# imazen/codec-eval

Hardware: AMD Instinct MI355X
Metric: metric MP/s (SSIMULACRA2+DSSIM+Butteraugli) at 1/2/4/8 GPU; HBM-roofline % (higher is better)
Workload: dtype f32

## Files before the change

### codec-eval_amd/csrc/ce_api.cpp

```cpp
#include <algorithm>
#include <atomic>
#include <condition_variable>
#include <functional>
#include <mutex>
#include <thread>
#include <cmath>
#include <cstdlib>
#include <cstring>
#include <new>

#include "ce_internal.h"

namespace {

thread_local std::string g_err_noctx;

int fail(ce_ctx *ctx, int code, const std::string &msg)
{
    if (ctx) ctx->err = msg; else g_err_noctx = msg;
    return code;
}

int bad_length(ce_ctx *ctx, size_t want, size_t got)
{
// ... 475 lines not shown
        if (b->h_stage[k]) hipHostFree(b->h_stage[k]);
        if (b->ev_stage[k]) hipEventDestroy(b->ev_stage[k]);
    }
    for (int l = 0; l < 3; l++) {
        if (b->metric_stream[l]) hipStreamSynchronize(b->metric_stream[l]);
        if (b->ev_join[l]) hipEventDestroy(b->ev_join[l]);
    }
    ce_ssim2_free(b);
    ce_dssim_free(b);
    ce_butteraugli_free(b);
    delete b;
}

static void invalidate_reference_state(ce_batch *b)
{
    b->ssim2_ref_src = nullptr;
    b->ds_ref_src = nullptr;
    b->ba_ref_src = nullptr;
    b->refs_rt_valid = false;
}

static bool is_pinned_host(const void *p)
{
    hipPointerAttribute_t a{};
    if (hipPointerGetAttributes(&a, p) != hipSuccess) {
        (void)hipGetLastError();
        return false;
    }
    return a.type == hipMemoryTypeHost;
}

// ... 530 lines not shown

int ce_batch_run(ce_batch *b, uint32_t n_pairs, uint32_t metric_mask, uint32_t flags, float intensity_target,
                 ce_scores *out)
{
    if (int rc = ce_batch_launch(b, n_pairs, metric_mask, flags, intensity_target)) return rc;
    return ce_batch_collect(b, n_pairs, out);
}


size_t ce_estimate_batch_bytes(uint32_t w, uint32_t h, uint32_t n_refs, uint32_t n_pairs, uint32_t metric_mask)
{
    const double px = (double)w * h, slots = (double)n_refs + n_pairs, pairs = n_pairs;
    double bytes = 3.0 * px * slots + 64.0 * pairs;
    double allocations = 8;
    if (metric_mask & CE_METRIC_SSIMULACRA2) {
        bytes += px * (20.0 * slots + 80.0 * pairs);
        allocations += 24;
    }
    if (metric_mask & CE_METRIC_DSSIM) {
        bytes += px * (6.0 * slots + 48.0 * n_refs + 17.4 * pairs);
        allocations += 24;
    }
    if (metric_mask & CE_METRIC_BUTTERAUGLI) {
        bytes += px * (91.0 * slots + 10.0 * n_refs + 1.0 * pairs);
        allocations += 20;
    }
    if (metric_mask & CE_METRIC_PSNR) bytes += 8.0 * pairs;
    return (size_t)(bytes * 1.2) + (size_t)(allocations * (256u << 10)) + (8u << 20);
}

size_t ce_estimate_batch_bytes_deep(uint32_t w, uint32_t h, uint32_t n_refs, uint32_t n_pairs, uint32_t metric_mask, uint32_t ref_depth,
                                    uint32_t test_depth)
// ... 770 lines not shown
```

### codec-eval_amd/csrc/ce_internal.h

```cpp
#pragma once

#include <hip/hip_runtime.h>

#include <cstdint>
#include <cstdio>
#include <map>
#include <string>
#include <tuple>
#include <utility>
#include <vector>

#include "ce_metrics.h"
#include "ce_metrics_debug.h"
#include "ce_plan.h"

#define CE_MAX_SCALES 6
#define CE_SSIM2_STREAMS 5
#define CE_DSSIM_SCALES 5
enum { CE_SRC_F32 = 0, CE_SRC_U8 = 1, CE_SRC_U16 = 2 };
static_assert(CE_MAX_SCALES == CE_SSIM2_MAX_SCALES, "the ABI's scale count is the pyramid's");

struct ce_scale_dims {
    uint32_t w, h, pitch;
    size_t plane;
// ... 90 lines not shown
    hipStream_t up_stream = nullptr;
    hipEvent_t ev_up = nullptr, ev_run = nullptr;
    bool uploads_pending = false, run_pending = false;
    bool inline_pending = false;
    bool counted_in_flight = false;
    uint8_t *h_wide[2] = {}, *d_wide[2] = {};
    hipEvent_t ev_wide[2] = {};
    bool wide_busy[2] = {};
    int next_wide = 0;

    int n_scales = 0;
    ce_scale_dims sd[CE_MAX_SCALES];
    float *d_lin[CE_MAX_SCALES] = {};
    float *d_xyb[CE_MAX_SCALES] = {};
    float *d_hbuf[CE_MAX_SCALES] = {};
    hipStream_t lvl_stream[CE_MAX_SCALES] = {};
    hipStream_t metric_stream[3] = {};
    hipEvent_t ev_fork = nullptr, ev_join[3] = {};
    hipEvent_t ev_prep[CE_MAX_SCALES] = {}, ev_done[CE_MAX_SCALES] = {};
    double *d_partials = nullptr;
    uint32_t max_vblocks = 0;
    double *d_avg = nullptr;
    float *s2_map = nullptr;
    float *s2_map_lvl[CE_MAX_SCALES] = {};
    uint32_t s2_map_pairs = 0, s2_norm_pairs = 0, s2_scales_run = 0;
    float *s2_cells = nullptr;
    size_t s2_cells_cap = 0;
    ce_dev_scores *d_scores = nullptr;
    ce_dev_scores *h_scores = nullptr;
    bool ssim2_ready = false;
    ce_xcd_list work_h, work_v;
    ce_xcd_list work_ht, work_vt;
    bool keep_ref_pyramid = false;
    const uint8_t *ssim2_ref_src = nullptr;
    uint32_t ssim2_ref_count = 0;
    int ssim2_ref_levels = 0;
    bool refs_rt_valid = false;
    int debug_max_scales = CE_MAX_SCALES;
    uint32_t ref_builds[3] = {0, 0, 0};

    struct dssim_level { uint32_t w, h, pitch; size_t plane; };
    int ds_levels = 0;
    dssim_level ds[CE_DSSIM_SCALES];
    float *ds_lin[2] = {};
    float *ds_img = nullptr;
    float *ds_rimg[CE_DSSIM_SCALES] = {}, *ds_rmu[CE_DSSIM_SCALES] = {}, *ds_rsq[CE_DSSIM_SCALES] = {};
    const uint8_t *ds_ref_src = nullptr;
    uint32_t ds_ref_count = 0;
    float *ds_map = nullptr;
    double *ds_part = nullptr;
    double *ds_level_scores = nullptr;
// ... 122 lines not shown
```

### codec-eval_amd/csrc/ce_plan.h

```cpp
#pragma once

#include <algorithm>
#include <cstdint>
#include <map>
#include <vector>

inline constexpr uint32_t ce_plan_ring_slots = 3;
inline constexpr size_t ce_plan_none = ~(size_t)0;

struct ce_plan_inputs {
    size_t budget;
    size_t per_pair;
    uint32_t pooled_pairs;
    size_t forced_chunks;
    size_t ramp;
};

struct ce_plan_chunk {
    uint32_t slot;
    uint32_t max_pairs;
    size_t collect_first;
    std::vector<std::vector<size_t>> refs;
};

// ... 27 lines not shown
        for (size_t p = bucket_begin; p < plan.size(); p++)
            if (plan[p].slot == c.slot) c.collect_first = p;
        plan.push_back(std::move(c));
    }
}

struct ce_plan_entry {
    uint32_t tile, pair;
};

struct ce_xcd_keys {
    uint32_t channels;
    uint32_t keys_per_channel;
    uint32_t tiles_per_key;
    uint32_t round_to = 1;
};

inline bool operator==(const ce_xcd_keys &a, const ce_xcd_keys &b)
{
    return a.channels == b.channels && a.keys_per_channel == b.keys_per_channel && a.tiles_per_key == b.tiles_per_key &&
           a.round_to == b.round_to;
}

inline std::vector<ce_plan_entry> ce_plan_xcd_list(const uint32_t *pair_ref, uint32_t n_pairs, uint32_t n_refs, const ce_xcd_keys &k)
{
    std::vector<std::vector<uint32_t>> pairs_of(n_refs);
    for (uint32_t p = 0; p < n_pairs; p++) pairs_of[pair_ref[p]].push_back(p);
    std::vector<ce_plan_entry> cls[8];
    uint32_t key = 0;
    for (const auto &pairs : pairs_of) {
        if (pairs.empty()) continue;
        for (uint32_t c = 0; c < k.channels; c++)
            for (uint32_t j = 0; j < k.keys_per_channel; j++, key++)
                for (uint32_t sub = 0; sub < k.tiles_per_key; sub++)
                    for (uint32_t p : pairs) cls[key & 7].push_back({(j * k.tiles_per_key + sub) | c << 16, p});
    }
    size_t len = 0;
    for (const auto &v : cls) len = std::max(len, v.size());
    len = (len + k.round_to - 1) / k.round_to * k.round_to;
    std::vector<ce_plan_entry> list(len * 8, ce_plan_entry{~0u, 0u});
    for (uint32_t x = 0; x < 8; x++)
        for (size_t i = 0; i < cls[x].size(); i++) list[i * 8 + x] = cls[x][i];
    return list;
}

inline uint32_t ce_plan_dssim_levels(uint32_t w, uint32_t h, uint32_t max_levels, uint32_t *level_w, uint32_t *level_h)
{
    if (w == 0 || h == 0) return 0;
    uint32_t n = 0;
    while (n < max_levels) {
// ... 26 lines not shown
```

### codec-eval_amd/csrc/ssim2.hip

```cpp
#include <algorithm>
#include <cstdlib>

#include "ce_internal.h"

namespace {

struct rg_consts {
    float mul_in[3];
    float mul_prev[3];
};

constexpr int kColsPerBlock = 64;

constexpr int kTailLevels = CE_MAX_SCALES - 1;
struct lvl_table {
    uint32_t n, first_level;
    uint32_t blk_end[kTailLevels];
    uint32_t w[kTailLevels], h[kTailLevels], pitch[kTailLevels];
    size_t plane[kTailLevels];
    const float *xyb[kTailLevels];
    float *hbuf[kTailLevels];
};

__device__ __forceinline__ uint32_t slot_of(uint32_t z, uint32_t n_refs_used, uint32_t max_refs)
{
    return z < n_refs_used ? z : max_refs + (z - n_refs_used);
}

__device__ __noinline__ float cbrt_f32_exact(float x)
{
    uint32_t hx = __float_as_uint(x) & 0x7fffffffu;
    if (hx == 0) return x;
    float t;
    if (hx < 0x00800000u) {
        t = __uint_as_float(0x4b800000u) * x;
        t = __uint_as_float((__float_as_uint(t) & 0x7fffffffu) / 3 + 642849266u);
// ... 283 lines not shown
                float *dst = base + l_dst[m];
                const bool rv = l_row[m] < h && col >= 0;
                dst[0] = (rv && col < (int)w) ? pf[m].x : 0.0f;
                dst[HB_LD] = (rv && col + 1 < (int)w) ? pf[m].y : 0.0f;
                dst[2 * HB_LD] = (rv && col + 2 < (int)w) ? pf[m].z : 0.0f;
                dst[3 * HB_LD] = (rv && col + 3 < (int)w) ? pf[m].w : 0.0f;
            }
        }
    };

    load_chunk(0);
    stash_chunk(0);
    if (n_chunks > 1) load_chunk(1);
    __syncthreads();

    const bool full = pair_first[p] == p;
    const uint32_t n_jobs = full ? CE_SSIM2_STREAMS : 3;
    const bool worker = tid < n_jobs * HB_ROWS;
    const uint32_t tj = worker ? tid / HB_ROWS : 0, tr = worker ? tid % HB_ROWS : 0;
    const uint32_t ts = full ? tj : (tj == 0 ? 1u : tj + 2u);
    const bool plain = ts < 2;
    const float *sp = &s_in[(ts == 1 || ts == 3) ? 1 : 0][tr];
    const float *sq = &s_in[(ts == 2) ? 0 : 1][tr];
    float *so = &s_out[ts * HB_HALF + tr];
    hblur_state st;
    st.p01 = st.q01 = hb_f2{0.0f, 0.0f};
    st.p2 = st.q2 = 0.0f;
#pragma unroll
    for (int j = 0; j < 10; j++) st.d[j] = 0.0f;
    float *obase = hbuf + ((size_t)p * 3 + c) * CE_SSIM2_STREAMS * plane;

// ... 16 lines not shown
                    *reinterpret_cast<float4 *>(obase + (size_t)os * plane + (size_t)(y0 + orow) * pitch + HB_CW * (k - 1) + 4 * oq) = v;
            }
        }
        lds_barrier();
    }
}

__device__ __forceinline__ double wave_sum(double v)
{
#pragma unroll
    for (int off = 32; off > 0; off >>= 1) v += __shfl_down(v, off, 64);
    return v;
}

constexpr int VB_G = 4;
constexpr int VB_PLANES = 7;
constexpr int VB_SLOT = VB_G * 64;
constexpr int VB_GROUP = VB_PLANES * VB_SLOT;

struct vblur_state {
    float prev[CE_SSIM2_STREAMS][3], prev2[CE_SSIM2_STREAMS][3];
    float rr[16][CE_SSIM2_STREAMS];
    double acc[6];
};

template <int GG, bool CHECKED, bool STORE>
__device__ __forceinline__ void vblur_group(vblur_state &st, const float *__restrict__ slot, int g, uint32_t h,
                                            const rg_consts &rg, float *__restrict__ map, uint32_t pitch, size_t plane,
                                            uint32_t lane, bool active)
{
    const float C2 = 0.0009f;
    float gacc[6] = {0.f, 0.f, 0.f, 0.f, 0.f, 0.f};
#pragma unroll
    for (int e = 0; e < VB_G; e++) {
        const uint32_t i = (uint32_t)(4 * g + e);
        constexpr int base = 4 * GG;
        const int re = base + e;
        float v[CE_SSIM2_STREAMS];
#pragma unroll
        for (int s = 0; s < CE_SSIM2_STREAMS; s++) {
            const float ld = slot[s * VB_SLOT + e * 64];
            const float right = (!CHECKED || i < h) ? ld : 0.0f;
            const float left = st.rr[(re + 6) & 15][s];
            st.rr[re][s] = right;
            v[s] = rg_step(left + right, st.prev[s], st.prev2[s], rg);
        }
        if (!CHECKED || (i >= 4 && i < h + 4)) {
            const float img1 = slot[5 * VB_SLOT + e * 64], img2 = slot[6 * VB_SLOT + e * 64];
            const float mu1 = v[0], mu2 = v[1], s11 = v[2], s22 = v[3], s12 = v[4];
            const float mu11 = mu1 * mu1, mu22 = mu2 * mu2, mu12 = mu1 * mu2;
            const float mu_diff = mu1 - mu2;
            const float num_m = __builtin_fmaf(mu_diff, -mu_diff, 1.0f);
            const float num_s = __builtin_fmaf(2.0f, s12 - mu12, C2);
            const float denom_s = (s11 - mu11) + (s22 - mu22) + C2;
            float d = 1.0f - (num_m * num_s) / denom_s;
            d = d > 0.0f ? d : 0.0f;
            const float dd = d * d;
            const float e1 = fabsf(img1 - mu1), e2 = fabsf(img2 - mu2);
            const float d1 = (e2 - e1) * __builtin_amdgcn_rcpf(1.0f + e1);
            const float artifact = d1 > 0.0f ? d1 : 0.0f;
            const float detail = d1 < 0.0f ? -d1 : 0.0f;
            const float aa = artifact * artifact, ll = detail * detail;
            if (STORE && active) {
                float *row = map + (size_t)(i - 4) * pitch;
// ... 1 lines not shown
                (row + plane)[lane] = artifact;
                (row + 2 * plane)[lane] = detail;
            }
            gacc[0] += d;
            gacc[1] += dd * dd;
            gacc[2] += artifact;
            gacc[3] += aa * aa;
            gacc[4] += detail;
            gacc[5] += ll * ll;
        }
    }
#pragma unroll
    for (int q = 0; q < 6; q++) st.acc[q] += (double)gacc[q];
}

struct ssim2_map_table {
    float *lvl[CE_MAX_SCALES];
};

template <int LEVEL, bool STORE>
__global__ __launch_bounds__(64) void k_ssim2_vblur_dma(const float *__restrict__ hbuf, const float *__restrict__ xyb,
                                                        const uint32_t *__restrict__ pair_ref,
                                                        double *__restrict__ partials, uint32_t w, uint32_t h,
                                                        uint32_t pitch, size_t plane, uint32_t max_refs, uint32_t scale,
                                                        uint32_t max_vblocks, rg_consts rg, lvl_table tab,
                                                        const uint2 *__restrict__ work, const uint32_t *__restrict__ pair_first,
                                                        ssim2_map_table maps)
{
    __shared__ __attribute__((aligned(16))) float ring[2 * VB_GROUP];
    uint32_t bx = blockIdx.x, c = blockIdx.y, p = blockIdx.z;
    if (work) {
        const uint2 wi = work[blockIdx.x];
        if (wi.x == ~0u) return;
        bx = wi.x & 0xffffu, c = wi.x >> 16, p = wi.y;
    }
    if (LEVEL < 0) {
        uint32_t l = 0;
        while (l + 1 < tab.n && bx >= tab.blk_end[l]) l++;
        bx -= l ? tab.blk_end[l - 1] : 0;
        xyb = tab.xyb[l], hbuf = tab.hbuf[l];
        w = tab.w[l], h = tab.h[l], pitch = tab.pitch[l], plane = tab.plane[l];
        scale = tab.first_level + l;
    }
    const uint32_t lane = threadIdx.x, x0 = bx * 64;
    const bool active = x0 + lane < w;
    const float *hb = hbuf + ((size_t)p * 3 + c) * CE_SSIM2_STREAMS * plane + x0;
    const float *hb_ref = hbuf + ((size_t)pair_first[p] * 3 + c) * CE_SSIM2_STREAMS * plane + x0;
    const float *xa = xyb + ((size_t)pair_ref[p] * 3 + c) * plane + x0;
    const float *xb = xyb + ((size_t)(max_refs + p) * 3 + c) * plane + x0;
    const uint32_t dr = lane >> 4, dc = (lane & 15) * 4;
    float *map = STORE ? maps.lvl[scale] + ((size_t)p * 9 + (size_t)c * 3) * plane + x0 : nullptr;

    using gptr = const __attribute__((address_space(1))) void *;
    using lptr = __attribute__((address_space(3))) void *;
    auto issue_group = [&](int g) {
        float *dst = ring + (g & 1) * VB_GROUP;
        const uint32_t row = min((uint32_t)(4 * g) + dr, h - 1);
        const size_t off = (size_t)row * pitch + dc;
#pragma unroll
        for (int s = 0; s < CE_SSIM2_STREAMS; s++)
            __builtin_amdgcn_global_load_lds((gptr)(((s == 0 || s == 2) ? hb_ref : hb) + (size_t)s * plane + off), (lptr)(dst + s * VB_SLOT), 16, 0, 0);
        const int rx = 4 * g - 4 + (int)dr;
        const size_t offx = (size_t)min((uint32_t)max(rx, 0), h - 1) * pitch + dc;
        __builtin_amdgcn_global_load_lds((gptr)(xa + offx), (lptr)(dst + 5 * VB_SLOT), 16, 0, 0);
        __builtin_amdgcn_global_load_lds((gptr)(xb + offx), (lptr)(dst + 6 * VB_SLOT), 16, 0, 0);
    };

    vblur_state st;
#pragma unroll
    for (int s = 0; s < CE_SSIM2_STREAMS; s++) {
#pragma unroll
        for (int k = 0; k < 3; k++) st.prev[s][k] = st.prev2[s][k] = 0.0f;
#pragma unroll
        for (int e = 0; e < 16; e++) st.rr[e][s] = 0.0f;
    }
#pragma unroll
    for (int q = 0; q < 6; q++) st.acc[q] = 0.0;
    const int n_groups = (int)((h + 4 + VB_G - 1) / VB_G);
    const int full_groups = (int)(h / VB_G);

    issue_group(0);
    issue_group(1);
#define CE_VGROUP(GG, CHECKED)                                                                         \
    do {                                                                                               \
                    \
        asm volatile("s_waitcnt vmcnt(7)" ::: "memory");                                               \
        vblur_group<GG, CHECKED, STORE>(st, ring + ((GG) & 1) * VB_GROUP + lane, g0 + (GG), h, rg, map, \
                                        pitch, plane, lane, active);                                   \
                      \
        asm volatile("s_waitcnt lgkmcnt(0)" ::: "memory");                                             \
        issue_group(g0 + (GG) + 2);                                                                    \
    } while (0)
    int g0 = 0;
    {
        CE_VGROUP(0, true);
        CE_VGROUP(1, true);
        if (2 < n_groups) CE_VGROUP(2, true);
        if (3 < n_groups) CE_VGROUP(3, true);
        g0 = 4;
    }
    for (; g0 + 3 < full_groups; g0 += 4) {
        CE_VGROUP(0, false);
        CE_VGROUP(1, false);
        CE_VGROUP(2, false);
        CE_VGROUP(3, false);
    }
    for (; g0 < n_groups; g0 += 4) {
        CE_VGROUP(0, true);
        if (g0 + 1 < n_groups) CE_VGROUP(1, true);
        if (g0 + 2 < n_groups) CE_VGROUP(2, true);
        if (g0 + 3 < n_groups) CE_VGROUP(3, true);
    }
#undef CE_VGROUP
    asm volatile("s_waitcnt vmcnt(0)" ::: "memory");
    double *dst = partials + ((((size_t)p * CE_MAX_SCALES + scale) * 3 + c) * max_vblocks + bx) * 6;
#pragma unroll
    for (int q = 0; q < 6; q++) {
        const double sum = wave_sum(active ? st.acc[q] : 0.0);
        if (lane == 0) dst[q] = sum;
    }
}

__global__ __launch_bounds__(256) void k_cbrt_sweep(uint32_t first, uint64_t count, unsigned long long *out)
{
    uint64_t mism = 0, slow = 0;
    for (uint64_t i = (uint64_t)blockIdx.x * blockDim.x + threadIdx.x; i < count; i += (uint64_t)gridDim.x * blockDim.x) {
        const float x = __uint_as_float(first + (uint32_t)i);
// ... 61 lines not shown
        else
            ssim = 100.0;
        scores[p].ssimulacra2 = ssim;
    }
}

}


void ce_ssim2_free(ce_batch *b)
{
    for (int s = 0; s < CE_MAX_SCALES; s++) {
        hipFree(b->d_lin[s]);
        hipFree(b->d_xyb[s]);
        hipFree(b->d_hbuf[s]);
        b->d_lin[s] = b->d_xyb[s] = b->d_hbuf[s] = nullptr;
        if (b->lvl_stream[s]) hipStreamSynchronize(b->lvl_stream[s]);
        if (b->ev_prep[s]) hipEventDestroy(b->ev_prep[s]);
        if (b->ev_done[s]) hipEventDestroy(b->ev_done[s]);
        b->lvl_stream[s] = nullptr;
        b->ev_prep[s] = b->ev_done[s] = nullptr;
    }
    hipFree(b->d_partials);
    hipFree(b->d_avg);
    hipFree(b->s2_map);
    hipFree(b->s2_cells);
    b->d_partials = nullptr;
    b->d_avg = nullptr;
    b->s2_map = b->s2_cells = nullptr;
    for (int s = 0; s < CE_MAX_SCALES; s++) b->s2_map_lvl[s] = nullptr;
    b->s2_cells_cap = 0;
    b->s2_map_pairs = b->s2_norm_pairs = 0;
    for (ce_xcd_list *L : {&b->work_h, &b->work_v, &b->work_ht, &b->work_vt}) ce_free_xcd_list(L);
    b->ssim2_ready = false;
}

static int ssim2_allocate(ce_batch *b)
{
    ce_ctx *ctx = b->ctx;
    const int ns = b->n_scales;
    const size_t slots = (size_t)b->max_refs + b->max_pairs;
    for (int s = 1; s < ns; s++)
        CE_HIP(ctx, hipMalloc(&b->d_lin[s], slots * 3 * b->sd[s].plane * sizeof(float)));
    for (int s = 0; s < ns; s++) {
        CE_HIP(ctx, hipMalloc(&b->d_xyb[s], slots * 3 * b->sd[s].plane * sizeof(float)));
        CE_HIP(ctx, hipMalloc(&b->d_hbuf[s], (size_t)b->max_pairs * 3 * CE_SSIM2_STREAMS * b->sd[s].plane * sizeof(float)));
        if (s == 0 && !(b->lvl_stream[0] = ce_ctx_aux_stream(ctx, ce_ctx::AUX_SSIM2_L0))) return CE_ERR_BACKEND;
        CE_HIP(ctx, hipEventCreateWithFlags(&b->ev_prep[s], hipEventDisableTiming));
        CE_HIP(ctx, hipEventCreateWithFlags(&b->ev_done[s], hipEventDisableTiming));
    }
    b->max_vblocks = (b->sd[0].w + kColsPerBlock - 1) / kColsPerBlock;
    CE_HIP(ctx, hipMalloc(&b->d_partials, (size_t)b->max_pairs * CE_MAX_SCALES * 3 * b->max_vblocks * 6 * sizeof(double)));
    CE_HIP(ctx, hipMalloc(&b->d_avg, (size_t)b->max_pairs * CE_MAX_SCALES * 18 * sizeof(double)));
    return CE_OK;
}

int ce_ssim2_prepare(ce_batch *b)
{
    if (b->ssim2_ready) return CE_OK;
    uint32_t sw[CE_MAX_SCALES], sh[CE_MAX_SCALES];
    const int ns = (int)ce_plan_ssim2_scales(b->w, b->h, CE_MAX_SCALES, sw, sh);
// ... 9 lines not shown
    }
    b->n_scales = ns;
    if (ns == 0) return CE_OK;
    const int rc = ssim2_allocate(b);
    if (rc != CE_OK) {
        const std::string why = b->ctx->err;
        ce_ssim2_free(b);
        (void)hipGetLastError();
        b->ctx->err = why;
        return rc;
    }
    b->ssim2_ready = true;
    return CE_OK;
}

static int build_pass_list(ce_batch *b, uint32_t n_pairs, uint32_t n_blocks, ce_xcd_list *L)
{
    if (n_blocks > 0xffffu) {
        b->ctx->err = "SSIMULACRA2: image too large for the block index of the work list";
        return CE_ERR_INVALID_ARG;
    }
    return ce_build_xcd_list(b, n_pairs, ce_xcd_keys{3, n_blocks, 1}, L);
}

int ce_launch_ssim2(ce_batch *b, const uint8_t *d_refs, uint32_t n_refs_used, uint32_t n_pairs, bool store_maps)
{
    ce_ctx *ctx = b->ctx;
    int rc = ce_ssim2_prepare(b);
    if (rc != CE_OK) return rc;
    ssim2_map_table maps{};
    if (store_maps) {
        if (!b->s2_map) {
            size_t total = 0;
            for (int s = 0; s < b->n_scales; s++) total += (size_t)b->max_pairs * 9 * b->sd[s].plane;
            if (hipMalloc(&b->s2_map, total * sizeof(float)) != hipSuccess) {
                b->s2_map = nullptr;
                (void)hipGetLastError();
// ... 3 lines not shown
            size_t off = 0;
            for (int s = 0; s < b->n_scales; s++) {
                b->s2_map_lvl[s] = b->s2_map + off;
                off += (size_t)b->max_pairs * 9 * b->sd[s].plane;
            }
        }
        for (int s = 0; s < b->n_scales; s++) maps.lvl[s] = b->s2_map_lvl[s];
    }
    rg_consts rg;
    ce_ssim2_recursive_gaussian(rg.mul_in, rg.mul_prev);
    const uint32_t n_slots = n_refs_used + n_pairs;
    const bool cached = b->keep_ref_pyramid && b->ssim2_ref_src == d_refs && b->ssim2_ref_count >= n_refs_used &&
                        b->ssim2_ref_levels == std::min(b->n_scales, b->debug_max_scales);
    const uint32_t z0 = cached ? n_refs_used : 0;
    if (!cached) b->ref_builds[0]++;
    using hblur_fn = void (*)(const float *, const uint32_t *, float *, uint32_t, uint32_t, uint32_t, size_t, uint32_t,
                              rg_consts, lvl_table, const uint2 *, const uint32_t *);
    using vblur_fn = void (*)(const float *, const float *, const uint32_t *, double *, uint32_t, uint32_t, uint32_t,
                              size_t, uint32_t, uint32_t, uint32_t, rg_consts, lvl_table, const uint2 *, const uint32_t *,
                              ssim2_map_table);
    const hblur_fn h_l0 = k_ssim2_hblur_lds<0>, h_tail = k_ssim2_hblur_lds<-1>;
    const vblur_fn v_l0 = k_ssim2_vblur_dma<0, false>, v_tail = k_ssim2_vblur_dma<-1, false>;
    const vblur_fn v_l0_map = k_ssim2_vblur_dma<0, true>, v_tail_map = k_ssim2_vblur_dma<-1, true>;
    scale_geom g{};
    const int levels = std::min(b->n_scales, b->debug_max_scales);
    hipStream_t s0 = ctx->prof_serial ? CE_STREAM(ctx) : b->lvl_stream[0];
    hipStream_t s1 = CE_STREAM(ctx);
    lvl_table tab{};
    lvl_table tab_v{};
    for (int s = 0; s < levels; s++) {
        const ce_scale_dims &d = b->sd[s];
        const bool has_next = s + 1 < levels;
        const ce_scale_dims &nd = b->sd[has_next ? s + 1 : s];
        const dim3 quad_grid(((d.w + 1) / 2 + 63) / 64, ((d.h + 1) / 2 + 3) / 4, n_slots - z0);
// ... 8 lines not shown
        else
            CE_LAUNCH(ctx, "ssim2_prep", k_ssim2_prep<CE_SRC_F32>, quad_grid, dim3(256), 0, d_refs, b->d_tests, ctx->d_lut_ssim2, ctx->d_lut_ssim2,
                      (const float *)b->d_lin[s], b->d_xyb[s], b->d_lin[has_next ? s + 1 : s], d.w, d.h, d.pitch, d.plane,
                      nd.pitch, nd.plane, has_next ? 1 : 0, b->img_bytes, n_refs_used, b->max_refs, z0);
        const uint32_t hblk = (d.h + HB_ROWS - 1) / HB_ROWS, vblk = (d.w + kColsPerBlock - 1) / kColsPerBlock;
        g.npix[s] = d.w * d.h;
        g.nblk[s] = vblk;
        if (s == 0) {
            if (s0 != CE_STREAM(ctx)) {
                CE_HIP(ctx, hipEventRecord(b->ev_prep[0], CE_STREAM(ctx)));
                CE_HIP(ctx, hipStreamWaitEvent(s0, b->ev_prep[0], 0));
            }
            if ((rc = build_pass_list(b, n_pairs, hblk, &b->work_h)) != CE_OK) return rc;
            if ((rc = build_pass_list(b, n_pairs, vblk, &b->work_v)) != CE_OK) return rc;
            CE_LAUNCH_ON(ctx, s0, "ssim2_hblur_L0", h_l0, dim3(b->work_h.len), dim3(HB_THREADS), 0, b->d_xyb[0], b->d_pair_ref,
                         b->d_hbuf[0], d.w, d.h, d.pitch, d.plane, b->max_refs, rg, tab, (const uint2 *)b->work_h.d,
                         (const uint32_t *)b->d_pair_first);
#define CE_VBLUR_L0_ARGS                                                                                                   \
    b->d_hbuf[0], b->d_xyb[0], b->d_pair_ref, b->d_partials, d.w, d.h, d.pitch, d.plane, b->max_refs, 0u, b->max_vblocks, rg, tab, \
        (const uint2 *)b->work_v.d, (const uint32_t *)b->d_pair_first, maps
            if (store_maps)
                CE_LAUNCH_ON(ctx, s0, "ssim2_vblur_ssim_map_L0", v_l0_map, dim3(b->work_v.len), dim3(64), 0, CE_VBLUR_L0_ARGS);
            else
                CE_LAUNCH_ON(ctx, s0, "ssim2_vblur_ssim_L0", v_l0, dim3(b->work_v.len), dim3(64), 0, CE_VBLUR_L0_ARGS);
#undef CE_VBLUR_L0_ARGS
            if (s0 != CE_STREAM(ctx)) CE_HIP(ctx, hipEventRecord(b->ev_done[0], s0));
        } else {
            const uint32_t l = tab.n++;
            tab_v.n = tab.n;
            tab.first_level = tab_v.first_level = 1;
            tab.blk_end[l] = (l ? tab.blk_end[l - 1] : 0) + hblk;
            tab_v.blk_end[l] = (l ? tab_v.blk_end[l - 1] : 0) + vblk;
            tab.w[l] = tab_v.w[l] = d.w;
            tab.h[l] = tab_v.h[l] = d.h;
            tab.pitch[l] = tab_v.pitch[l] = d.pitch;
            tab.plane[l] = tab_v.plane[l] = d.plane;
            tab.xyb[l] = tab_v.xyb[l] = b->d_xyb[s];
            tab.hbuf[l] = tab_v.hbuf[l] = b->d_hbuf[s];
        }
    }
    if (tab.n) {
        if (s1 != CE_STREAM(ctx)) {
            CE_HIP(ctx, hipEventRecord(b->ev_prep[1], CE_STREAM(ctx)));
            CE_HIP(ctx, hipStreamWaitEvent(s1, b->ev_prep[1], 0));
        }
        if ((rc = build_pass_list(b, n_pairs, tab.blk_end[tab.n - 1], &b->work_ht)) != CE_OK) return rc;
        if ((rc = build_pass_list(b, n_pairs, tab_v.blk_end[tab_v.n - 1], &b->work_vt)) != CE_OK) return rc;
        CE_LAUNCH_ON(ctx, s1, "ssim2_hblur_L1-5", h_tail, dim3(b->work_ht.len), dim3(HB_THREADS), 0,
                     (const float *)nullptr, b->d_pair_ref, (float *)nullptr, 0u, 0u, 0u, (size_t)0, b->max_refs, rg, tab,
                     (const uint2 *)b->work_ht.d, (const uint32_t *)b->d_pair_first);
#define CE_VBLUR_TAIL_ARGS                                                                                                  \
    (const float *)nullptr, (const float *)nullptr, b->d_pair_ref, b->d_partials, 0u, 0u, 0u, (size_t)0, b->max_refs, 0u,        \
        b->max_vblocks, rg, tab_v, (const uint2 *)b->work_vt.d, (const uint32_t *)b->d_pair_first, maps
        if (store_maps)
            CE_LAUNCH_ON(ctx, s1, "ssim2_vblur_ssim_map_L1-5", v_tail_map, dim3(b->work_vt.len), dim3(64), 0, CE_VBLUR_TAIL_ARGS);
        else
            CE_LAUNCH_ON(ctx, s1, "ssim2_vblur_ssim_L1-5", v_tail, dim3(b->work_vt.len), dim3(64), 0, CE_VBLUR_TAIL_ARGS);
#undef CE_VBLUR_TAIL_ARGS
        if (s1 != CE_STREAM(ctx)) CE_HIP(ctx, hipEventRecord(b->ev_done[1], s1));
    }
    if (s0 != CE_STREAM(ctx)) {
        CE_HIP(ctx, hipStreamWaitEvent(CE_STREAM(ctx), b->ev_done[0], 0));
        if (tab.n && s1 != CE_STREAM(ctx)) CE_HIP(ctx, hipStreamWaitEvent(CE_STREAM(ctx), b->ev_done[1], 0));
    }
    if (b->keep_ref_pyramid && !cached) {
        b->ssim2_ref_src = d_refs;
        b->ssim2_ref_count = n_refs_used;
        b->ssim2_ref_levels = levels;
    }
    CE_LAUNCH(ctx, "ssim2_finalize", k_ssim2_finalize, dim3(n_pairs), dim3(128), 0, b->d_partials, b->d_avg,
              b->d_scores, (uint32_t)levels, b->max_vblocks, g);
    CE_HIP(ctx, hipGetLastError());
    return CE_OK;
}

int ce_ssim2_cbrt_sweep(ce_ctx *ctx, uint32_t first_bits, uint64_t count, uint64_t *mismatches, uint64_t *slow_path)
{
    unsigned long long *d = nullptr, h[2] = {0, 0};
    CE_HIP(ctx, hipMalloc(&d, sizeof(h)));
    CE_HIP(ctx, hipMemsetAsync(d, 0, sizeof(h), ctx->stream));
    CE_LAUNCH(ctx, "cbrt_sweep", k_cbrt_sweep, dim3(4096), dim3(256), 0, first_bits, count, d);
    CE_HIP(ctx, hipMemcpyAsync(h, d, sizeof(h), hipMemcpyDeviceToHost, ctx->stream));
    CE_HIP(ctx, hipStreamSynchronize(ctx->stream));
// ... 32 lines not shown
```

Measured before the change: 19040.

## Precompute reference-side vertical blurs once per reference and reuse across pairs

Adds a per-reference vertical-blur kernel that writes the reference's blurred mu and sigma11 planes into a new refcol buffer, launched once per reference rather than once per pair. The main SSIM vblur kernel then blurs only three test-dependent streams and loads the reference columns precomputed. The refcol buffers are cached across calls when the reference pyramid is kept, so the horizontal blur can skip the reference streams. This removes redundant reference blurring for multi-pair references, at the cost of extra memory, an extra launch, and host-side bookkeeping.

```diff
diff --git a/codec-eval_amd/csrc/ce_api.cpp b/codec-eval_amd/csrc/ce_api.cpp
--- a/codec-eval_amd/csrc/ce_api.cpp
+++ b/codec-eval_amd/csrc/ce_api.cpp
@@ -513,7 +513,7 @@
 
 static void invalidate_reference_state(ce_batch *b)
 {
-    b->ssim2_ref_src = nullptr;
+    b->ssim2_ref_src = b->ssim2_refcol_src = nullptr;
     b->ds_ref_src = nullptr;
     b->ba_ref_src = nullptr;
     b->refs_rt_valid = false;
@@ -1074,8 +1074,8 @@
     double bytes = 3.0 * px * slots + 64.0 * pairs;
     double allocations = 8;
     if (metric_mask & CE_METRIC_SSIMULACRA2) {
-        bytes += px * (20.0 * slots + 80.0 * pairs);
-        allocations += 24;
+        bytes += px * (20.0 * slots + 80.0 * pairs + 32.0 * n_refs);
+        allocations += 30;
     }
     if (metric_mask & CE_METRIC_DSSIM) {
         bytes += px * (6.0 * slots + 48.0 * n_refs + 17.4 * pairs);
diff --git a/codec-eval_amd/csrc/ce_internal.h b/codec-eval_amd/csrc/ce_internal.h
--- a/codec-eval_amd/csrc/ce_internal.h
+++ b/codec-eval_amd/csrc/ce_internal.h
@@ -128,6 +128,7 @@
     float *d_lin[CE_MAX_SCALES] = {};
     float *d_xyb[CE_MAX_SCALES] = {};
     float *d_hbuf[CE_MAX_SCALES] = {};
+    float *d_refcol[CE_MAX_SCALES] = {};
     hipStream_t lvl_stream[CE_MAX_SCALES] = {};
     hipStream_t metric_stream[3] = {};
     hipEvent_t ev_fork = nullptr, ev_join[3] = {};
@@ -143,12 +144,14 @@
     ce_dev_scores *d_scores = nullptr;
     ce_dev_scores *h_scores = nullptr;
     bool ssim2_ready = false;
-    ce_xcd_list work_h, work_v;
-    ce_xcd_list work_ht, work_vt;
+    ce_xcd_list work_h, work_v, work_r;
+    ce_xcd_list work_ht, work_vt, work_rt;
     bool keep_ref_pyramid = false;
     const uint8_t *ssim2_ref_src = nullptr;
     uint32_t ssim2_ref_count = 0;
     int ssim2_ref_levels = 0;
+    const uint8_t *ssim2_refcol_src = nullptr;
+    std::vector<uint8_t> ssim2_refcol_has;
     bool refs_rt_valid = false;
     int debug_max_scales = CE_MAX_SCALES;
     uint32_t ref_builds[3] = {0, 0, 0};
diff --git a/codec-eval_amd/csrc/ce_plan.h b/codec-eval_amd/csrc/ce_plan.h
--- a/codec-eval_amd/csrc/ce_plan.h
+++ b/codec-eval_amd/csrc/ce_plan.h
@@ -65,12 +65,13 @@
     uint32_t keys_per_channel;
     uint32_t tiles_per_key;
     uint32_t round_to = 1;
+    bool first_pair_only = false;
 };
 
 inline bool operator==(const ce_xcd_keys &a, const ce_xcd_keys &b)
 {
     return a.channels == b.channels && a.keys_per_channel == b.keys_per_channel && a.tiles_per_key == b.tiles_per_key &&
-           a.round_to == b.round_to;
+           a.round_to == b.round_to && a.first_pair_only == b.first_pair_only;
 }
 
 inline std::vector<ce_plan_entry> ce_plan_xcd_list(const uint32_t *pair_ref, uint32_t n_pairs, uint32_t n_refs, const ce_xcd_keys &k)
@@ -84,7 +85,10 @@
         for (uint32_t c = 0; c < k.channels; c++)
             for (uint32_t j = 0; j < k.keys_per_channel; j++, key++)
                 for (uint32_t sub = 0; sub < k.tiles_per_key; sub++)
-                    for (uint32_t p : pairs) cls[key & 7].push_back({(j * k.tiles_per_key + sub) | c << 16, p});
+                    for (uint32_t p : pairs) {
+                        cls[key & 7].push_back({(j * k.tiles_per_key + sub) | c << 16, p});
+                        if (k.first_pair_only) break;
+                    }
     }
     size_t len = 0;
     for (const auto &v : cls) len = std::max(len, v.size());
diff --git a/codec-eval_amd/csrc/ssim2.hip b/codec-eval_amd/csrc/ssim2.hip
--- a/codec-eval_amd/csrc/ssim2.hip
+++ b/codec-eval_amd/csrc/ssim2.hip
@@ -20,6 +20,7 @@
     size_t plane[kTailLevels];
     const float *xyb[kTailLevels];
     float *hbuf[kTailLevels];
+    float *refcol[kTailLevels];
 };
 
 __device__ __forceinline__ uint32_t slot_of(uint32_t z, uint32_t n_refs_used, uint32_t max_refs)
@@ -333,7 +334,7 @@
     if (n_chunks > 1) load_chunk(1);
     __syncthreads();
 
-    const bool full = pair_first[p] == p;
+    const bool full = pair_first && pair_first[p] == p;
     const uint32_t n_jobs = full ? CE_SSIM2_STREAMS : 3;
     const bool worker = tid < n_jobs * HB_ROWS;
     const uint32_t tj = worker ? tid / HB_ROWS : 0, tr = worker ? tid % HB_ROWS : 0;
@@ -380,18 +381,51 @@
 }
 
 constexpr int VB_G = 4;
+constexpr int VB_STREAMS = 3;
 constexpr int VB_PLANES = 7;
 constexpr int VB_SLOT = VB_G * 64;
 constexpr int VB_GROUP = VB_PLANES * VB_SLOT;
-
+constexpr int VR_STREAMS = 2;
+constexpr int VR_GROUP = VR_STREAMS * VB_SLOT;
+
+template <int NS>
 struct vblur_state {
-    float prev[CE_SSIM2_STREAMS][3], prev2[CE_SSIM2_STREAMS][3];
-    float rr[16][CE_SSIM2_STREAMS];
+    float prev[NS][3], prev2[NS][3];
+    float rr[16][NS];
     double acc[6];
 };
 
+template <int NS>
+__device__ __forceinline__ void vblur_clear(vblur_state<NS> &st)
+{
+#pragma unroll
+    for (int s = 0; s < NS; s++) {
+#pragma unroll
+        for (int k = 0; k < 3; k++) st.prev[s][k] = st.prev2[s][k] = 0.0f;
+#pragma unroll
+        for (int e = 0; e < 16; e++) st.rr[e][s] = 0.0f;
+    }
+#pragma unroll
+    for (int q = 0; q < 6; q++) st.acc[q] = 0.0;
+}
+
+template <int GG, bool CHECKED, int NS>
+__device__ __forceinline__ void vblur_step(vblur_state<NS> &st, const float *__restrict__ slot, int e, uint32_t i, uint32_t h,
+                                           const rg_consts &rg, float (&v)[NS])
+{
+    const int re = 4 * GG + e;
+#pragma unroll
+    for (int s = 0; s < NS; s++) {
+        const float ld = slot[s * VB_SLOT + e * 64];
+        const float right = (!CHECKED || i < h) ? ld : 0.0f;
+        const float left = st.rr[(re + 6) & 15][s];
+        st.rr[re][s] = right;
+        v[s] = rg_step(left + right, st.prev[s], st.prev2[s], rg);
+    }
+}
+
 template <int GG, bool CHECKED, bool STORE>
-__device__ __forceinline__ void vblur_group(vblur_state &st, const float *__restrict__ slot, int g, uint32_t h,
+__device__ __forceinline__ void vblur_group(vblur_state<VB_STREAMS> &st, const float *__restrict__ slot, int g, uint32_t h,
                                             const rg_consts &rg, float *__restrict__ map, uint32_t pitch, size_t plane,
                                             uint32_t lane, bool active)
 {
@@ -400,20 +434,12 @@
 #pragma unroll
     for (int e = 0; e < VB_G; e++) {
         const uint32_t i = (uint32_t)(4 * g + e);
-        constexpr int base = 4 * GG;
-        const int re = base + e;
-        float v[CE_SSIM2_STREAMS];
-#pragma unroll
-        for (int s = 0; s < CE_SSIM2_STREAMS; s++) {
-            const float ld = slot[s * VB_SLOT + e * 64];
-            const float right = (!CHECKED || i < h) ? ld : 0.0f;
-            const float left = st.rr[(re + 6) & 15][s];
-            st.rr[re][s] = right;
-            v[s] = rg_step(left + right, st.prev[s], st.prev2[s], rg);
-        }
+        float v[VB_STREAMS];
+        vblur_step<GG, CHECKED>(st, slot, e, i, h, rg, v);
         if (!CHECKED || (i >= 4 && i < h + 4)) {
             const float img1 = slot[5 * VB_SLOT + e * 64], img2 = slot[6 * VB_SLOT + e * 64];
-            const float mu1 = v[0], mu2 = v[1], s11 = v[2], s22 = v[3], s12 = v[4];
+            const float mu1 = slot[3 * VB_SLOT + e * 64], s11 = slot[4 * VB_SLOT + e * 64];
+            const float mu2 = v[0], s22 = v[1], s12 = v[2];
             const float mu11 = mu1 * mu1, mu22 = mu2 * mu2, mu12 = mu1 * mu2;
             const float mu_diff = mu1 - mu2;
             const float num_m = __builtin_fmaf(mu_diff, -mu_diff, 1.0f);
@@ -445,73 +471,162 @@
     for (int q = 0; q < 6; q++) st.acc[q] += (double)gacc[q];
 }
 
+template <int GG, bool CHECKED>
+__device__ __forceinline__ void vref_group(vblur_state<VR_STREAMS> &st, const float *__restrict__ slot, int g, uint32_t h,
+                                           const rg_consts &rg, float *__restrict__ out, uint32_t pitch, size_t plane,
+                                           uint32_t lane, bool active)
+{
+#pragma unroll
+    for (int e = 0; e < VB_G; e++) {
+        const uint32_t i = (uint32_t)(4 * g + e);
+        float v[VR_STREAMS];
+        vblur_step<GG, CHECKED>(st, slot, e, i, h, rg, v);
+        if ((!CHECKED || (i >= 4 && i < h + 4)) && active) {
+            float *row = out + (size_t)(i - 4) * pitch;
+            row[lane] = v[0];
+            (row + plane)[lane] = v[1];
+        }
+    }
+}
+
+#define CE_VBLUR_WALK(VGROUP)                                  \
+    do {                                                       \
+        int g0 = 0;                                            \
+        {                                                      \
+            VGROUP(0, true);                                   \
+            VGROUP(1, true);                                   \
+            if (2 < n_groups) VGROUP(2, true);                 \
+            if (3 < n_groups) VGROUP(3, true);                 \
+            g0 = 4;                                            \
+        }                                                      \
+        for (; g0 + 3 < full_groups; g0 += 4) {                \
+            VGROUP(0, false);                                  \
+            VGROUP(1, false);                                  \
+            VGROUP(2, false);                                  \
+            VGROUP(3, false);                                  \
+        }                                                      \
+        for (; g0 < n_groups; g0 += 4) {                       \
+            VGROUP(0, true);                                   \
+            if (g0 + 1 < n_groups) VGROUP(1, true);            \
+            if (g0 + 2 < n_groups) VGROUP(2, true);            \
+            if (g0 + 3 < n_groups) VGROUP(3, true);            \
+        }                                                      \
+    } while (0)
+
+using vb_gptr = const __attribute__((address_space(1))) void *;
+using vb_lptr = __attribute__((address_space(3))) void *;
+
+template <int LEVEL>
+__global__ __launch_bounds__(64) void k_ssim2_vblur_ref(const float *__restrict__ hbuf, float *__restrict__ refcol,
+                                                        const uint32_t *__restrict__ pair_ref, uint32_t w, uint32_t h,
+                                                        uint32_t pitch, size_t plane, rg_consts rg, lvl_table tab,
+                                                        const uint2 *__restrict__ work)
+{
+    __shared__ __attribute__((aligned(16))) float ring[2 * VR_GROUP];
+    const uint2 wi = work[blockIdx.x];
+    if (wi.x == ~0u) return;
+    uint32_t bx = wi.x & 0xffffu;
+    const uint32_t c = wi.x >> 16, p = wi.y;
+    if (LEVEL < 0) {
+        uint32_t l = 0;
+        while (l + 1 < tab.n && bx >= tab.blk_end[l]) l++;
+        bx -= l ? tab.blk_end[l - 1] : 0;
+        hbuf = tab.hbuf[l], refcol = tab.refcol[l];
+        w = tab.w[l], h = tab.h[l], pitch = tab.pitch[l], plane = tab.plane[l];
+    }
+    const uint32_t lane = threadIdx.x, x0 = bx * 64;
+    const bool active = x0 + lane < w;
+    const float *hb = hbuf + ((size_t)p * 3 + c) * CE_SSIM2_STREAMS * plane + x0;
+    float *out = refcol + ((size_t)pair_ref[p] * 3 + c) * VR_STREAMS * plane + x0;
+    const uint32_t dr = lane >> 4, dc = (lane & 15) * 4;
+
+    auto issue_group = [&](int g) {
+        float *dst = ring + (g & 1) * VR_GROUP;
+        const size_t off = (size_t)min((uint32_t)(4 * g) + dr, h - 1) * pitch + dc;
+        __builtin_amdgcn_global_load_lds((vb_gptr)(hb + off), (vb_lptr)dst, 16, 0, 0);
+        __builtin_amdgcn_global_load_lds((vb_gptr)(hb + 2 * plane + off), (vb_lptr)(dst + VB_SLOT), 16, 0, 0);
+    };
+
+    vblur_state<VR_STREAMS> st;
+    vblur_clear(st);
+    const int n_groups = (int)((h + 4 + VB_G - 1) / VB_G);
+    const int full_groups = (int)(h / VB_G);
+
+    issue_group(0);
+    issue_group(1);
+#define CE_VGROUP(GG, CHECKED)                                                                         \
+    do {                                                                                               \
+                                  \
+        asm volatile("s_waitcnt vmcnt(2)" ::: "memory");                                               \
+        vref_group<GG, CHECKED>(st, ring + ((GG) & 1) * VR_GROUP + lane, g0 + (GG), h, rg, out, pitch, \
+                                plane, lane, active);                                                  \
+                      \
+        asm volatile("s_waitcnt lgkmcnt(0)" ::: "memory");                                             \
+        issue_group(g0 + (GG) + 2);                                                                    \
+    } while (0)
+    CE_VBLUR_WALK(CE_VGROUP);
+#undef CE_VGROUP
+    asm volatile("s_waitcnt vmcnt(0)" ::: "memory");
+}
+
 struct ssim2_map_table {
     float *lvl[CE_MAX_SCALES];
 };
 
 template <int LEVEL, bool STORE>
 __global__ __launch_bounds__(64) void k_ssim2_vblur_dma(const float *__restrict__ hbuf, const float *__restrict__ xyb,
+                                                        const float *__restrict__ refcol,
                                                         const uint32_t *__restrict__ pair_ref,
                                                         double *__restrict__ partials, uint32_t w, uint32_t h,
                                                         uint32_t pitch, size_t plane, uint32_t max_refs, uint32_t scale,
                                                         uint32_t max_vblocks, rg_consts rg, lvl_table tab,
-                                                        const uint2 *__restrict__ work, const uint32_t *__restrict__ pair_first,
-                                                        ssim2_map_table maps)
+                                                        const uint2 *__restrict__ work, ssim2_map_table maps)
 {
     __shared__ __attribute__((aligned(16))) float ring[2 * VB_GROUP];
-    uint32_t bx = blockIdx.x, c = blockIdx.y, p = blockIdx.z;
-    if (work) {
-        const uint2 wi = work[blockIdx.x];
-        if (wi.x == ~0u) return;
-        bx = wi.x & 0xffffu, c = wi.x >> 16, p = wi.y;
-    }
+    const uint2 wi = work[blockIdx.x];
+    if (wi.x == ~0u) return;
+    uint32_t bx = wi.x & 0xffffu;
+    const uint32_t c = wi.x >> 16, p = wi.y;
     if (LEVEL < 0) {
         uint32_t l = 0;
         while (l + 1 < tab.n && bx >= tab.blk_end[l]) l++;
         bx -= l ? tab.blk_end[l - 1] : 0;
-        xyb = tab.xyb[l], hbuf = tab.hbuf[l];
+        xyb = tab.xyb[l], hbuf = tab.hbuf[l], refcol = tab.refcol[l];
         w = tab.w[l], h = tab.h[l], pitch = tab.pitch[l], plane = tab.plane[l];
         scale = tab.first_level + l;
     }
     const uint32_t lane = threadIdx.x, x0 = bx * 64;
     const bool active = x0 + lane < w;
     const float *hb = hbuf + ((size_t)p * 3 + c) * CE_SSIM2_STREAMS * plane + x0;
-    const float *hb_ref = hbuf + ((size_t)pair_first[p] * 3 + c) * CE_SSIM2_STREAMS * plane + x0;
+    const float *rc = refcol + ((size_t)pair_ref[p] * 3 + c) * VR_STREAMS * plane + x0;
     const float *xa = xyb + ((size_t)pair_ref[p] * 3 + c) * plane + x0;
     const float *xb = xyb + ((size_t)(max_refs + p) * 3 + c) * plane + x0;
     const uint32_t dr = lane >> 4, dc = (lane & 15) * 4;
     float *map = STORE ? maps.lvl[scale] + ((size_t)p * 9 + (size_t)c * 3) * plane + x0 : nullptr;
 
-    using gptr = const __attribute__((address_space(1))) void *;
-    using lptr = __attribute__((address_space(3))) void *;
     auto issue_group = [&](int g) {
         float *dst = ring + (g & 1) * VB_GROUP;
         const uint32_t row = min((uint32_t)(4 * g) + dr, h - 1);
         const size_t off = (size_t)row * pitch + dc;
-#pragma unroll
-        for (int s = 0; s < CE_SSIM2_STREAMS; s++)
-            __builtin_amdgcn_global_load_lds((gptr)(((s == 0 || s == 2) ? hb_ref : hb) + (size_t)s * plane + off), (lptr)(dst + s * VB_SLOT), 16, 0, 0);
+        __builtin_amdgcn_global_load_lds((vb_gptr)(hb + 1 * plane + off), (vb_lptr)(dst + 0 * VB_SLOT), 16, 0, 0);
+        __builtin_amdgcn_global_load_lds((vb_gptr)(hb + 3 * plane + off), (vb_lptr)(dst + 1 * VB_SLOT), 16, 0, 0);
+        __builtin_amdgcn_global_load_lds((vb_gptr)(hb + 4 * plane + off), (vb_lptr)(dst + 2 * VB_SLOT), 16, 0, 0);
         const int rx = 4 * g - 4 + (int)dr;
         const size_t offx = (size_t)min((uint32_t)max(rx, 0), h - 1) * pitch + dc;
-        __builtin_amdgcn_global_load_lds((gptr)(xa + offx), (lptr)(dst + 5 * VB_SLOT), 16, 0, 0);
-        __builtin_amdgcn_global_load_lds((gptr)(xb + offx), (lptr)(dst + 6 * VB_SLOT), 16, 0, 0);
+        __builtin_amdgcn_global_load_lds((vb_gptr)(rc + offx), (vb_lptr)(dst + 3 * VB_SLOT), 16, 0, 0);
+        __builtin_amdgcn_global_load_lds((vb_gptr)(rc + plane + offx), (vb_lptr)(dst + 4 * VB_SLOT), 16, 0, 0);
+        __builtin_amdgcn_global_load_lds((vb_gptr)(xa + offx), (vb_lptr)(dst + 5 * VB_SLOT), 16, 0, 0);
+        __builtin_amdgcn_global_load_lds((vb_gptr)(xb + offx), (vb_lptr)(dst + 6 * VB_SLOT), 16, 0, 0);
     };
 
-    vblur_state st;
-#pragma unroll
-    for (int s = 0; s < CE_SSIM2_STREAMS; s++) {
-#pragma unroll
-        for (int k = 0; k < 3; k++) st.prev[s][k] = st.prev2[s][k] = 0.0f;
-#pragma unroll
-        for (int e = 0; e < 16; e++) st.rr[e][s] = 0.0f;
-    }
-#pragma unroll
-    for (int q = 0; q < 6; q++) st.acc[q] = 0.0;
+    vblur_state<VB_STREAMS> st;
+    vblur_clear(st);
     const int n_groups = (int)((h + 4 + VB_G - 1) / VB_G);
     const int full_groups = (int)(h / VB_G);
 
     issue_group(0);
     issue_group(1);
+    static_assert(VB_PLANES == 7, "the vmcnt below is the number of DMA requests of one group");
 #define CE_VGROUP(GG, CHECKED)                                                                         \
     do {                                                                                               \
                     \
@@ -522,26 +637,7 @@
         asm volatile("s_waitcnt lgkmcnt(0)" ::: "memory");                                             \
         issue_group(g0 + (GG) + 2);                                                                    \
     } while (0)
-    int g0 = 0;
-    {
-        CE_VGROUP(0, true);
-        CE_VGROUP(1, true);
-        if (2 < n_groups) CE_VGROUP(2, true);
-        if (3 < n_groups) CE_VGROUP(3, true);
-        g0 = 4;
-    }
-    for (; g0 + 3 < full_groups; g0 += 4) {
-        CE_VGROUP(0, false);
-        CE_VGROUP(1, false);
-        CE_VGROUP(2, false);
-        CE_VGROUP(3, false);
-    }
-    for (; g0 < n_groups; g0 += 4) {
-        CE_VGROUP(0, true);
-        if (g0 + 1 < n_groups) CE_VGROUP(1, true);
-        if (g0 + 2 < n_groups) CE_VGROUP(2, true);
-        if (g0 + 3 < n_groups) CE_VGROUP(3, true);
-    }
+    CE_VBLUR_WALK(CE_VGROUP);
 #undef CE_VGROUP
     asm volatile("s_waitcnt vmcnt(0)" ::: "memory");
     double *dst = partials + ((((size_t)p * CE_MAX_SCALES + scale) * 3 + c) * max_vblocks + bx) * 6;
@@ -633,7 +729,8 @@
         hipFree(b->d_lin[s]);
         hipFree(b->d_xyb[s]);
         hipFree(b->d_hbuf[s]);
-        b->d_lin[s] = b->d_xyb[s] = b->d_hbuf[s] = nullptr;
+        hipFree(b->d_refcol[s]);
+        b->d_lin[s] = b->d_xyb[s] = b->d_hbuf[s] = b->d_refcol[s] = nullptr;
         if (b->lvl_stream[s]) hipStreamSynchronize(b->lvl_stream[s]);
         if (b->ev_prep[s]) hipEventDestroy(b->ev_prep[s]);
         if (b->ev_done[s]) hipEventDestroy(b->ev_done[s]);
@@ -650,7 +747,8 @@
     for (int s = 0; s < CE_MAX_SCALES; s++) b->s2_map_lvl[s] = nullptr;
     b->s2_cells_cap = 0;
     b->s2_map_pairs = b->s2_norm_pairs = 0;
-    for (ce_xcd_list *L : {&b->work_h, &b->work_v, &b->work_ht, &b->work_vt}) ce_free_xcd_list(L);
+    for (ce_xcd_list *L : {&b->work_h, &b->work_v, &b->work_r, &b->work_ht, &b->work_vt, &b->work_rt}) ce_free_xcd_list(L);
+    b->ssim2_refcol_src = nullptr;
     b->ssim2_ready = false;
 }
 
@@ -664,6 +762,7 @@
     for (int s = 0; s < ns; s++) {
         CE_HIP(ctx, hipMalloc(&b->d_xyb[s], slots * 3 * b->sd[s].plane * sizeof(float)));
         CE_HIP(ctx, hipMalloc(&b->d_hbuf[s], (size_t)b->max_pairs * 3 * CE_SSIM2_STREAMS * b->sd[s].plane * sizeof(float)));
+        CE_HIP(ctx, hipMalloc(&b->d_refcol[s], (size_t)b->max_refs * 3 * VR_STREAMS * b->sd[s].plane * sizeof(float)));
         if (s == 0 && !(b->lvl_stream[0] = ce_ctx_aux_stream(ctx, ce_ctx::AUX_SSIM2_L0))) return CE_ERR_BACKEND;
         CE_HIP(ctx, hipEventCreateWithFlags(&b->ev_prep[s], hipEventDisableTiming));
         CE_HIP(ctx, hipEventCreateWithFlags(&b->ev_done[s], hipEventDisableTiming));
@@ -703,13 +802,13 @@
     return CE_OK;
 }
 
-static int build_pass_list(ce_batch *b, uint32_t n_pairs, uint32_t n_blocks, ce_xcd_list *L)
+static int build_pass_list(ce_batch *b, uint32_t n_pairs, uint32_t n_blocks, ce_xcd_list *L, bool per_reference = false)
 {
     if (n_blocks > 0xffffu) {
         b->ctx->err = "SSIMULACRA2: image too large for the block index of the work list";
         return CE_ERR_INVALID_ARG;
     }
-    return ce_build_xcd_list(b, n_pairs, ce_xcd_keys{3, n_blocks, 1}, L);
+    return ce_build_xcd_list(b, n_pairs, ce_xcd_keys{3, n_blocks, 1, 1, per_reference}, L);
 }
 
 int ce_launch_ssim2(ce_batch *b, const uint8_t *d_refs, uint32_t n_refs_used, uint32_t n_pairs, bool store_maps)
@@ -743,10 +842,15 @@
                         b->ssim2_ref_levels == std::min(b->n_scales, b->debug_max_scales);
     const uint32_t z0 = cached ? n_refs_used : 0;
     if (!cached) b->ref_builds[0]++;
+    std::vector<uint8_t> has_pair(n_refs_used, 0);
+    for (uint32_t p = 0; p < n_pairs; p++) has_pair[b->h_pair_ref[p]] = 1;
+    bool refcol_cached = cached && b->ssim2_refcol_src == d_refs && b->ssim2_refcol_has.size() >= n_refs_used;
+    for (uint32_t r = 0; refcol_cached && r < n_refs_used; r++) refcol_cached = !has_pair[r] || b->ssim2_refcol_has[r];
+    const uint32_t *d_first = refcol_cached ? nullptr : (const uint32_t *)b->d_pair_first;
     using hblur_fn = void (*)(const float *, const uint32_t *, float *, uint32_t, uint32_t, uint32_t, size_t, uint32_t,
                               rg_consts, lvl_table, const uint2 *, const uint32_t *);
-    using vblur_fn = void (*)(const float *, const float *, const uint32_t *, double *, uint32_t, uint32_t, uint32_t,
-                              size_t, uint32_t, uint32_t, uint32_t, rg_consts, lvl_table, const uint2 *, const uint32_t *,
+    using vblur_fn = void (*)(const float *, const float *, const float *, const uint32_t *, double *, uint32_t, uint32_t,
+                              uint32_t, size_t, uint32_t, uint32_t, uint32_t, rg_consts, lvl_table, const uint2 *,
                               ssim2_map_table);
     const hblur_fn h_l0 = k_ssim2_hblur_lds<0>, h_tail = k_ssim2_hblur_lds<-1>;
     const vblur_fn v_l0 = k_ssim2_vblur_dma<0, false>, v_tail = k_ssim2_vblur_dma<-1, false>;
@@ -785,11 +889,16 @@
             if ((rc = build_pass_list(b, n_pairs, hblk, &b->work_h)) != CE_OK) return rc;
             if ((rc = build_pass_list(b, n_pairs, vblk, &b->work_v)) != CE_OK) return rc;
             CE_LAUNCH_ON(ctx, s0, "ssim2_hblur_L0", h_l0, dim3(b->work_h.len), dim3(HB_THREADS), 0, b->d_xyb[0], b->d_pair_ref,
-                         b->d_hbuf[0], d.w, d.h, d.pitch, d.plane, b->max_refs, rg, tab, (const uint2 *)b->work_h.d,
-                         (const uint32_t *)b->d_pair_first);
+                         b->d_hbuf[0], d.w, d.h, d.pitch, d.plane, b->max_refs, rg, tab, (const uint2 *)b->work_h.d, d_first);
+            if (!refcol_cached) {
+                if ((rc = build_pass_list(b, n_pairs, vblk, &b->work_r, true)) != CE_OK) return rc;
+                CE_LAUNCH_ON(ctx, s0, "ssim2_vblur_ref_L0", k_ssim2_vblur_ref<0>, dim3(b->work_r.len), dim3(64), 0,
+                             (const float *)b->d_hbuf[0], b->d_refcol[0], (const uint32_t *)b->d_pair_ref, d.w, d.h, d.pitch, d.plane,
+                             rg, tab, (const uint2 *)b->work_r.d);
+            }
 #define CE_VBLUR_L0_ARGS                                                                                                   \
-    b->d_hbuf[0], b->d_xyb[0], b->d_pair_ref, b->d_partials, d.w, d.h, d.pitch, d.plane, b->max_refs, 0u, b->max_vblocks, rg, tab, \
-        (const uint2 *)b->work_v.d, (const uint32_t *)b->d_pair_first, maps
+    b->d_hbuf[0], b->d_xyb[0], b->d_refcol[0], b->d_pair_ref, b->d_partials, d.w, d.h, d.pitch, d.plane, b->max_refs, 0u,  \
+        b->max_vblocks, rg, tab, (const uint2 *)b->work_v.d, maps
             if (store_maps)
                 CE_LAUNCH_ON(ctx, s0, "ssim2_vblur_ssim_map_L0", v_l0_map, dim3(b->work_v.len), dim3(64), 0, CE_VBLUR_L0_ARGS);
             else
@@ -808,6 +917,7 @@
             tab.plane[l] = tab_v.plane[l] = d.plane;
             tab.xyb[l] = tab_v.xyb[l] = b->d_xyb[s];
             tab.hbuf[l] = tab_v.hbuf[l] = b->d_hbuf[s];
+            tab.refcol[l] = tab_v.refcol[l] = b->d_refcol[s];
         }
     }
     if (tab.n) {
@@ -819,10 +929,16 @@
         if ((rc = build_pass_list(b, n_pairs, tab_v.blk_end[tab_v.n - 1], &b->work_vt)) != CE_OK) return rc;
         CE_LAUNCH_ON(ctx, s1, "ssim2_hblur_L1-5", h_tail, dim3(b->work_ht.len), dim3(HB_THREADS), 0,
                      (const float *)nullptr, b->d_pair_ref, (float *)nullptr, 0u, 0u, 0u, (size_t)0, b->max_refs, rg, tab,
-                     (const uint2 *)b->work_ht.d, (const uint32_t *)b->d_pair_first);
+                     (const uint2 *)b->work_ht.d, d_first);
+        if (!refcol_cached) {
+            if ((rc = build_pass_list(b, n_pairs, tab_v.blk_end[tab_v.n - 1], &b->work_rt, true)) != CE_OK) return rc;
+            CE_LAUNCH_ON(ctx, s1, "ssim2_vblur_ref_L1-5", k_ssim2_vblur_ref<-1>, dim3(b->work_rt.len), dim3(64), 0,
+                         (const float *)nullptr, (float *)nullptr, (const uint32_t *)b->d_pair_ref, 0u, 0u, 0u, (size_t)0, rg, tab_v,
+                         (const uint2 *)b->work_rt.d);
+        }
 #define CE_VBLUR_TAIL_ARGS                                                                                                  \
-    (const float *)nullptr, (const float *)nullptr, b->d_pair_ref, b->d_partials, 0u, 0u, 0u, (size_t)0, b->max_refs, 0u,        \
-        b->max_vblocks, rg, tab_v, (const uint2 *)b->work_vt.d, (const uint32_t *)b->d_pair_first, maps
+    (const float *)nullptr, (const float *)nullptr, (const float *)nullptr, b->d_pair_ref, b->d_partials, 0u, 0u, 0u, (size_t)0, \
+        b->max_refs, 0u, b->max_vblocks, rg, tab_v, (const uint2 *)b->work_vt.d, maps
         if (store_maps)
             CE_LAUNCH_ON(ctx, s1, "ssim2_vblur_ssim_map_L1-5", v_tail_map, dim3(b->work_vt.len), dim3(64), 0, CE_VBLUR_TAIL_ARGS);
         else
@@ -838,6 +954,10 @@
         b->ssim2_ref_src = d_refs;
         b->ssim2_ref_count = n_refs_used;
         b->ssim2_ref_levels = levels;
+    }
+    if (b->keep_ref_pyramid && !refcol_cached) {
+        b->ssim2_refcol_src = d_refs;
+        b->ssim2_refcol_has = has_pair;
     }
     CE_LAUNCH(ctx, "ssim2_finalize", k_ssim2_finalize, dim3(n_pairs), dim3(128), 0, b->d_partials, b->d_avg,
               b->d_scores, (uint32_t)levels, b->max_vblocks, g);
```

Result: no change. 19020 (median of 2 runs) (-0.1%).
